# Sudaraka88/LDWeaver

Measured on AMD Instinct MI355X. Metric: MI SNP-pairs/sec, higher is better.
Workload: dtype i8

## Files before the change

ldweaver_amd/csrc/ldw_api.hip:

```cpp
#include <algorithm>
#include <atomic>
#include <chrono>
#include <cmath>
#include <cstdio>
#include <cstdlib>
#include <cstring>

#include <thread>
#include "ldw_internal.h"
#include "ldw_dev.h"
#include "ldw_fasta.h"
#include "ldw_links_read.h"
#include "ldw_slots.h"

namespace ldw {
int check_gpu(ldw_ctx *ctx) {
    LDW_REQUIRE(ctx != nullptr, LDW_ERR_ARG, "null context");
    LDW_HIP(hipSetDevice(ctx->device));
    return LDW_OK;
}
}

using namespace ldw;

// ... 811 lines not shown
            for (int y = 0; y < kb; ++y) {
                const double q = (phi[x] == y ? p[x] : 0.0) + 0.5;
                const double D = p[x] * pY[y] + rxy + p[x] * rX + pY[y] * rY;
                if (!(D > 0.0)) return 1e300;
                F += q * log(q * den / D);
            }
        F /= den;
        if (!(F == F)) return 1e300;
        best = F > best ? F : best;
    }
    return best;
}

__global__ __launch_bounds__(256) void k_snp_sup(int64_t L, const uint32_t *__restrict__ slot_meta, const int64_t *__restrict__ slot_pfix,
                                                 const double *__restrict__ r, double scale, double neff, double r_min, double *__restrict__ sup) {
    const int64_t a = (int64_t)blockIdx.x * 256 + threadIdx.x;
    if (a >= L) return;
    const uint32_t m = slot_meta[a];
    const int n = (int)(m & 7), ka = n + 1;
    double out[4] = {1e300, 1e300, 1e300, 1e300};
    const uint32_t full = (2u << n) - 1u;
    if ((ka == 2 || ka == 3) && ((m >> 3) & full) == full && r[a] == (double)ka) {
        double p[3] = {0.0, 0.0, 0.0};
        double minor = 0.0;
        for (int x = 0; x < ka; ++x) {
            p[x] = (double)slot_pfix[a * 5 + x] * scale;
            if (x < n) minor += p[x];
        }
        if (minor < 0.05 * neff + 4.0)
            for (int kb = 2; kb <= 3; ++kb) {
                out[kb - 2] = mi_vertex_sup(p, ka, kb, neff, 0.25 * ka * kb) * (1.0 + 1e-12) + 1e-12;
                const double rfloor = 0.25 * r_min * r_min;
                out[2 + kb - 2] = mi_vertex_sup(p, ka, kb, neff, rfloor < 0.25 * ka * kb ? rfloor : 0.25 * ka * kb) * (1.0 + 1e-12) + 1e-12;
            }
    }
    for (int k = 0; k < 4; ++k) sup[a * 4 + k] = out[k];
}

static int slot_marginals(ldw_ctx *c, const std::vector<int64_t> &w, int shift, ldw::DevBuf &dst, const char *what) {
    const int64_t L = c->L, Npad = c->Npad;
    ldw::DevBuf d_w, d_p, d_cnt;
    if (int rc = d_w.reserve((size_t)Npad * 8)) return rc;
    if (int rc = d_p.reserve((size_t)L * 40)) return rc;
    if (int rc = d_cnt.reserve((size_t)L * 20)) return rc;
    if (int rc = dst.reserve((size_t)L * 40)) return rc;
    hipError_t he = hipMemcpyAsync(d_w.p, w.data(), (size_t)Npad * 8, hipMemcpyHostToDevice, c->stream);
    hipLaunchKernelGGL(k_counts_marginals, dim3((unsigned)((L + 3) / 4)), dim3(256), 0, c->stream, c->states.as<uint8_t>(), L, Npad, d_w.as<int64_t>(),
                       d_cnt.as<int32_t>(), d_p.as<int64_t>());
    std::vector<int64_t> by_state((size_t)L * 5), by_slot((size_t)L * 5, 0);
    if (he == hipSuccess) he = hipMemcpyAsync(by_state.data(), d_p.p, (size_t)L * 40, hipMemcpyDeviceToHost, c->stream);
    if (he == hipSuccess) he = hipStreamSynchronize(c->stream);
    if (he != hipSuccess) return ldw::hip_fail(he, what, __FILE__, __LINE__);
    for (int64_t a = 0; a < L; ++a) {
        const uint32_t m = c->rows.h_slot_meta[a];
        const int n = (int)(m & 7);
        for (int i = 0; i <= n; ++i) by_slot[a * 5 + i] = by_state[a * 5 + ((m >> (8 + 3 * i)) & 7)] >> shift;
    }
// ... 81 lines not shown
    const int64_t R = c->rows.R;
    lap("slot maps built on the host");
    if (int rc = c->rows.row0.reserve((size_t)(L + 1) * 4)) return rc;
    if (int rc = c->rows.slot_meta.reserve((size_t)L * 4)) return rc;
    if (int rc = c->rows.Mbits.reserve((size_t)(R + TILE) * c->KW * 8)) return rc;
    if (int rc = c->small.reserve((size_t)(R + 1) * 4)) return rc;
    LDW_HIP(hipMemcpyAsync(c->rows.row0.p, c->rows.h_row0.data(), (size_t)(L + 1) * 4, hipMemcpyHostToDevice, c->stream));
    LDW_HIP(hipMemcpyAsync(c->rows.slot_meta.p, meta.data(), (size_t)L * 4, hipMemcpyHostToDevice, c->stream));
    LDW_HIP(hipMemcpyAsync(c->rows.slot_pfix.p, spf.data(), (size_t)L * 40, hipMemcpyHostToDevice, c->stream));
    if (c->apx.apx_ok) {
        if (int rc = slot_marginals(c, c->apx.h_vapx, c->apx.apx_e_last, c->rows.slot_papx, "approximate-weight marginals")) return rc;
    }
    LDW_HIP(hipMemsetAsync(c->rows.Mbits.as<uint64_t>() + (size_t)R * c->KW, 0, (size_t)TILE * c->KW * 8, c->stream));
    lap("approximate marginals");
    if (R > 0) {
        LDW_HIP(hipMemcpyAsync(c->small.p, rowinfo.data(), (size_t)R * 4, hipMemcpyHostToDevice, c->stream));
        LDW_REQUIRE(R < 2147483647LL, LDW_ERR_ARG, "too many indicator rows");
        if (int rc = fill_rows_bits(c, c->small.as<int32_t>(), R)) return rc;
    }
    if (int rc = c->rows.snp_sup.reserve((size_t)L * 32)) return rc;
    hipLaunchKernelGGL(k_snp_sup, dim3((unsigned)((L + 255) / 256)), dim3(256), 0, c->stream, L, c->rows.slot_meta.as<uint32_t>(), c->rows.slot_pfix.as<int64_t>(),
                       c->meta.r.as<double>(), std::ldexp(1.0, -c->wts.frac_bits), c->wts.neff, c->meta.r_min, c->rows.snp_sup.as<double>());
    LDW_HIP(hipGetLastError());
    LDW_HIP(hipStreamSynchronize(c->stream));
    lap("bit rows + per-SNP bounds");
    c->rows_rebuilt();
    return LDW_OK;
}

}
```

ldweaver_amd/csrc/ldw_apx.h:

```cpp
#pragma once
#include "ldw_internal.h"
#include "ldw_epi.h"

namespace ldw {

struct PopSeg {
    uint32_t mask;
    uint32_t flush;
    int64_t V;
};

constexpr int APX_TW = 128;
struct ApxGemmArgs {
    const uint64_t *panel_t, *panel_f;
    int RTpad, RFpad, M2;
    const uint8_t *dig_a, *dig_b;
    const int32_t *shift;
    int32_t *G;
    int lower_only;
    int fine;
    int fuse;
    const uint8_t *bin_t, *bin_f;
    const int2 *tab;
    int tab_nb;
    uint8_t *clean;
    const uint8_t *sr_mask;
    unsigned long long *skip_ctr;
    uint32_t *tile_list;
    unsigned int *n_live;
    int grid_wgs;
    const uint8_t *rflag_t, *rflag_f;
    struct ApxMaybe *maybe;
    unsigned int *maybe_n;
    unsigned int maybe_cap;
};
int launch_pack_panel(ldw_ctx *c, const int32_t *rowlist, int Rpad, uint64_t *panel, hipStream_t st, const int32_t *rowlist2 = nullptr, int Rpad2 = 0,
                      uint64_t *panel2 = nullptr);
int launch_apx_live_tiles(ldw_ctx *c, const ApxGemmArgs &P, hipStream_t st);
int launch_gemm_apx(ldw_ctx *c, const ApxGemmArgs &P, hipStream_t st);
int apx_run_grid(const ldw_ctx *c, int RTpad, int RFpad);
enum PairForm : int { PAIR_FORM_AUTO = 0, PAIR_FORM_QUARTER = 1, PAIR_FORM_WAVE_LDS = 2, PAIR_FORM_WAVE_GLOBAL = 3, PAIR_FORM_BITS = 4 };
struct PairSumsRan {
    int form = 0;
    bool lds160 = false;
};
int launch_pair_sums(ldw_ctx *c, const EpiArgs &A, int64_t *sums, hipStream_t st, int form, int grid_wgs, PairSumsRan *ran);
int launch_pairs_exact(ldw_ctx *c, const EpiArgs &A, unsigned long long *ghist, int64_t *sums, hipStream_t st);

}
```

ldweaver_amd/csrc/ldw_apx.hip:

```cpp
#include <algorithm>
#include <cmath>
#include <cstdlib>
#include <cstring>

#include "ldw_apx.h"
#include "ldw_dev.h"

using namespace ldw;

namespace ldw {

namespace {
constexpr int64_t APX_PROD_CAP = 12000;
struct ProdTable {
    std::vector<int32_t> val;
    std::vector<uint8_t> a, b;
    ProdTable() {
        std::vector<std::pair<int32_t, std::pair<uint8_t, uint8_t>>> all;
        for (int x = 0; x <= 127; ++x)
            for (int y = x; y <= 127; ++y) all.push_back({x * y, {(uint8_t)x, (uint8_t)y}});
        std::sort(all.begin(), all.end());
        for (auto &e : all)
            if (val.empty() || val.back() != e.first) {
                val.push_back(e.first);
// ... 303 lines not shown
            S.fand &= a & 0xFFu;
            S.forr |= o & 0xFFu;
        }
    }
    return S;
}

__global__ __launch_bounds__(256) void k_apx_live_tiles(ApxGemmArgs P) {
    constexpr int MT = APX_MT, NT = 2, TH = 32 * MT, TWd = 32 * NT;
    __shared__ unsigned int s_wave[4], s_base;
    const int ty = (int)blockIdx.x, ntx = P.RFpad / TWd;
    const int lane = threadIdx.x & 63, wave = threadIdx.x >> 6;
    const TileSummary T = apx_fold_rows(P.bin_t + (int64_t)ty * TH, P.rflag_t ? P.rflag_t + (int64_t)ty * TH : nullptr, TH);
    unsigned int n_pruned = 0;
    for (int tx0 = 0; tx0 < ntx; tx0 += 256) {
        const int tx = tx0 + (int)threadIdx.x;
        const bool valid = tx < ntx && !(P.lower_only && tx * TWd + TWd - 1 < ty * TH);
        bool pruned = false, all_binned = false;
        if (valid && !(P.sr_mask && P.sr_mask[(int64_t)((ty * TH) / 128) * (P.RFpad / 64) + tx] != 0)) {
            const TileSummary F = apx_fold_rows(P.bin_f + (int64_t)tx * TWd, P.rflag_f ? P.rflag_f + (int64_t)tx * TWd : nullptr, TWd);
            all_binned = T.bmax < P.tab_nb && F.bmax < P.tab_nb;
            if (P.rflag_t) {
                const unsigned kt = T.fand & PF_KIND, kf = F.fand & PF_KIND;
                pruned = kt >= 2u && kt == (T.forr & PF_KIND) && kf >= 2u && kf == (F.forr & PF_KIND) &&
                         ((T.fand & (kf == 2u ? PF_DEAD2 : PF_DEAD3)) != 0u || (F.fand & (kt == 2u ? PF_DEAD2 : PF_DEAD3)) != 0u);
            }
            if (!pruned && all_binned && (T.bmax - T.bmin + 1) * (F.bmax - F.bmin + 1) <= 64) {
                bool ok = true;
                for (int bt = T.bmin; bt <= T.bmax; ++bt)
                    for (int bf = F.bmin; bf <= F.bmax; ++bf) {
                        const int2 th = P.tab[bt * P.tab_nb + bf];
                        ok = ok && th.x < 0 && th.y == 2147483647;
                    }
                pruned = ok;
            }
        }
        if (pruned && all_binned) {
#pragma unroll
            for (int i = 0; i < MT; ++i)
#pragma unroll
                for (int h = 0; h < (NT * 32) / 64; ++h) P.clean[(int64_t)((ty * TH + 32 * i) / 32) * (P.RFpad / 64) + (tx * TWd) / 64 + h] = 1;
        }
        const bool live = valid && !pruned;
        const unsigned long long lm = __ballot(live);
        n_pruned += (unsigned int)__popcll(__ballot(valid && pruned));
        if (lane == 0) s_wave[wave] = (unsigned int)__popcll(lm);
        __syncthreads();
        if (threadIdx.x == 0) {
// ... 872 lines not shown
```

ldweaver_amd/csrc/ldw_internal.h:

```cpp
#pragma once
#include <hip/hip_runtime.h>
#include <stdint.h>
#include <stdlib.h>
#include <algorithm>
#include <string>
#include <atomic>
#include <chrono>
#include <memory>
#include <mutex>
#include <thread>
#include <vector>

#include "../../include/ldweaver_amd.h"
#include "../../include/ldweaver_amd_debug.h"
#include "ldw_own.h"

#define LDW_NSLOT 3


namespace ldw {

void set_error(const char *fmt, ...);
int hip_fail(hipError_t e, const char *what, const char *file, int line);

// ... 111 lines not shown
        int64_t n_slots = 0;
    } pos_ord;
    void drop() { have_meta = pos_only = false; }
    void mark_set(bool positions_only) { have_meta = true, pos_only = positions_only; }
    void set_positions(const int32_t *POS_, int64_t L) {
        h_POS.assign(POS_, POS_ + L);
        pos_sorted = true;
        for (int64_t i = 1; i < L && pos_sorted; ++i) pos_sorted = POS_[i] >= POS_[i - 1];
        pos_strict = pos_sorted;
        for (int64_t i = 1; i < L && pos_strict; ++i) pos_strict = POS_[i] > POS_[i - 1];
        pos_ord.n_slots = 0;
    }
};

struct SrSizing {
    double sr_total_dist = -1;
    int64_t sr_total = -1;
    uint64_t sr_share_key = 0;
    int64_t sr_share_rows = -1;
    void learn_share(uint64_t key, int64_t n_rows) { sr_share_key = key, sr_share_rows = n_rows; }
    void forget() { sr_total = sr_share_rows = -1, sr_total_dist = -1; }
};

struct OrderCache { std::vector<int32_t> idx, order; };
struct RowMap {
    bool rows_ready = false;
    int64_t R = 0;
    DevBuf Mbits;
    DevBuf row0;
    DevBuf slot_meta;
    DevBuf slot_pfix;
    DevBuf slot_pfix_hi;
    bool hi_ready = false;
    DevBuf slot_papx;
    DevBuf counts;
    DevBuf pfix_state;
    DevBuf snp_sup;
    std::vector<int32_t> h_row0;
    std::vector<uint32_t> h_slot_meta;
    std::vector<int32_t> h_counts;
    std::vector<int64_t> h_minor_w;
    std::vector<int32_t> h_span_bad;
    std::mutex order_mtx;
    std::vector<std::unique_ptr<OrderCache>> order_cache;
    void invalidate() { rows_ready = false; }
    void rebuilt() { rows_ready = true, hi_ready = false, order_cache.clear(); }
};

struct Speculation {
    bool spec_seen[2] = {false, false};
    bool spec_probed[2] = {false, false};
    int spec_hist[2][6] = {{0, 0, 0, 0, 0, 0}, {0, 0, 0, 0, 0, 0}};
    int spec_hist_n[2] = {0, 0};
    bool spec_small[2] = {false, false};
    int spec_B_next[2] = {-1, -1};
    bool maybe_off = false;
    DevBuf tab11[2];
    double tab11_lo[2] = {0, 0};
    int tab11_cur[2] = {0, 0};
    float tab11_c = 0;
// ... 20 lines not shown
};

struct PassCounters {
    int64_t apx_blocks = 0, apx_units_listed = 0, apx_pairs_listed = 0, probe_blocks = 0, generic_blocks = 0;
    int64_t form_launches[5] = {0, 0, 0, 0, 0};
    int64_t pair_kernel_launches[2] = {0, 0};
    int64_t apx_waves_skipped = 0, apx_waves_total = 0;
    int64_t tab11_builds = 0;
    int64_t slot_grown = 0;
    int64_t maybe_entries = 0;
    int64_t pair_list_overflows = 0, maybe_overflows = 0;
    int64_t span_items = 0, span_blocks = 0, span_fallbacks = 0;
    std::atomic<int64_t> sorted_blocks{0};
    int64_t spec_misses = 0, blocks_run = 0, screen_violations = 0, mixed_blocks = 0;
    double gemm_stat[6] = {0, 0, 0, 0, 0, 0};
};

struct Knobs {
    int engine = LDW_ENGINE_MFMA;
    int path_mode = 0;
    int select_mode = 0;
    int mixed = 1;
    bool prune = true;
    bool span_on = true;
    int span_max = 8;
    bool overlap = true;
    int screen = 1;
};

inline bool host_timing() {
    static const bool on = getenv("LDW_HOST_TIMING") != nullptr;
    return on;
}
struct HostClock {
    using Point = std::chrono::steady_clock::time_point;
    static Point now() { return std::chrono::steady_clock::now(); }
    static double ms(Point a, Point b) { return std::chrono::duration<double, std::milli>(b - a).count(); }
    static double us(Point a, Point b) { return std::chrono::duration<double, std::micro>(b - a).count(); }
};
}

struct ldw_ctx {
    int device = 0;
    int n_cu = 0;
    ldw::Stream stream;
    ldw::Stream copy_stream, gemm_stream;
// ... 139 lines not shown
```

ldweaver_amd/csrc/ldw_mi.hip:

```cpp
#include <algorithm>
#include <chrono>
#include <cmath>
#include <cstring>
#include "ldw_prim.h"

#include "ldw_internal.h"
#include "ldw_dev.h"
#ifndef LDW_SCREEN_V
#define LDW_SCREEN_V 2
#endif
#ifndef LDW_SCREEN_WAVES
#define LDW_SCREEN_WAVES 6
#endif
#include "ldw_epi.h"
#include "ldw_pass_plan.h"
#include <future>

#include "ldw_apx.h"

using namespace ldw;

namespace ldw {
#include "ldw_mi_screen.inc"
#include "ldw_mi_eval.inc"
#include "ldw_mi_select.inc"
}

namespace {
#include "ldw_mi_block.inc"
#include "ldw_mi_items.inc"
#include "ldw_mi_pass.inc"
}

namespace ldw {
int ensure_streams(ldw_ctx *c) {
    if (c->streams_ready) return LDW_OK;
    const unsigned quiet = hipEventDisableTiming;
    LDW_HIP(c->copy_stream.ensure(hipStreamNonBlocking));
// ... 124 lines not shown
        if ((rc = c->G.reserve((size_t)RFpad * RTpad * 8))) break;
        for (int pass = 0; pass < 2 && rc == LDW_OK; ++pass) {
            int64_t *host_out = pass == 0 ? counts_out : fixed_out;
            if (!host_out) continue;
            rc = launch_gemm_bits(c, c->rows.Mbits.as<uint64_t>(), c->KW, c->rowlist_t.as<int32_t>(), RTpad, c->rowlist_f.as<int32_t>(), RFpad, c->G.as<int64_t>(),
                                  pass == 0 ? 1 : c->wts.nlimbs, pass == 0 ? d_ones.as<int8_t>() : c->wts.digits.as<int8_t>(), 0);
            if (rc) break;
            hipLaunchKernelGGL(k_tables, dim3((unsigned)((n + 63) / 64)), dim3(64), 0, c->stream, c->G.as<int64_t>(), RFpad,
                               c->idx_f.as<int32_t>(), c->lrow_f.as<int32_t>(), c->idx_t.as<int32_t>(),
                               c->lrow_t.as<int32_t>(), (int)n, c->rows.slot_meta.as<uint32_t>(),
                               pass == 0 ? d_cmarg.as<int64_t>() : c->rows.slot_pfix.as<int64_t>(), d_out.as<int64_t>());
            he = hipMemcpyAsync(host_out + p0 * 25, d_out.p, (size_t)n * 25 * 8, hipMemcpyDeviceToHost, c->stream);
            if (he == hipSuccess) he = hipStreamSynchronize(c->stream);
            if (he != hipSuccess) rc = ldw::hip_fail(he, "joint tables copy", __FILE__, __LINE__);
        }
    }
    return rc;
}

int ldw_links_begin(ldw_ctx *c, int64_t nblocks_capacity) {
    if (int rc = check_gpu(c)) return rc;
    if (int rc = join_prepare(c)) return rc;
    LDW_REQUIRE(nblocks_capacity > 0, LDW_ERR_ARG, "ldw_links_begin: capacity must be positive");
    if (c->links.blk_capacity != 0) {
        if (c->gemm_stream) LDW_HIP(hipStreamSynchronize(c->gemm_stream));
        if (c->copy_stream) LDW_HIP(hipStreamSynchronize(c->copy_stream));
        LDW_HIP(hipStreamSynchronize(c->stream));
        c->links.blk_capacity = 0;
    }
    if (int rc = ensure_rows(c)) return rc;
    const size_t need = 64 + (size_t)LDW_NSLOT * LDW_SPAN_MAX * PICK_STRIDE + (size_t)nblocks_capacity * 32 + 64;
    if (int rc = c->small.reserve(need)) return rc;
    LDW_HIP(hipMemsetAsync(c->small.p, 0, need, c->stream));
    if (int rc = ensure_streams(c)) return rc;
    LDW_HIP(hipEventRecord(c->ev_up[0], c->stream));
    LDW_HIP(hipStreamWaitEvent(c->gemm_stream, c->ev_up[0], 0));
    while ((int64_t)c->ev_pool.size() < nblocks_capacity * EVB) {
        ldw::Event e;
        LDW_HIP(e.ensure());
        c->ev_pool.push_back(std::move(e));
    }
    for (int k = 0; k < LDW_NSLOT; ++k) c->done_recorded[k] = false;
    c->early_sr = false;
    c->ev_valid.assign((size_t)nblocks_capacity, 1);
    c->lrc_recorded = false;
    c->links.new_pass();
// ... 376 lines not shown
```

ldweaver_amd/csrc/ldw_mi_block.inc:

```

int upload_i32(ldw_ctx *c, ldw::DevBuf &buf, const std::vector<int32_t> &v) {
    if (int rc = buf.reserve(v.size() * 4 + 4)) return rc;
    if (!v.empty()) LDW_HIP(hipMemcpyAsync(buf.p, v.data(), v.size() * 4, hipMemcpyHostToDevice, c->stream));
    return LDW_OK;
}

struct SideLists {
    std::vector<int32_t> rowlist, lrow, pos;
    std::vector<uint8_t> cls;
    int Rpad = 0;
};

int build_side(ldw_ctx *c, const int32_t *idx, int64_t n, SideLists &S, const std::vector<int32_t> *order1 = nullptr) {
    S.lrow.assign((size_t)n, 0);
    S.rowlist.clear();
    S.pos.clear();
    S.cls.clear();
    const int32_t zero_row = (int32_t)c->rows.R;
    for (int64_t k = 0; k < n; ++k)
        LDW_REQUIRE(idx[k] >= 0 && idx[k] < c->L, LDW_ERR_ARG, "SNP index %d out of range 0..%lld", idx[k], (long long)c->L - 1);
    for (int cl : {1, 2, 4}) {
        const bool ordered = cl == 1 && order1 != nullptr;
        const int64_t cnt = ordered ? (int64_t)order1->size() : n;
        for (int64_t kk = 0; kk < cnt; ++kk) {
            const int64_t k = ordered ? (int64_t)(*order1)[(size_t)kk] : kk;
            const int32_t a = idx[k];
            const int nr = c->rows.h_row0[a + 1] - c->rows.h_row0[a];
            const int mine = nr <= 1 ? 1 : (nr == 2 ? 2 : 4);
            if (mine != cl) continue;
            S.lrow[k] = (int32_t)S.rowlist.size();
            for (int q = 0; q < cl; ++q) {
                S.rowlist.push_back(q < nr ? c->rows.h_row0[a] + q : zero_row);
                S.pos.push_back(q == 0 ? (int32_t)k : -1);
            }
        }
        while (S.rowlist.size() % 32) {
            S.rowlist.push_back(zero_row);
            S.pos.push_back(-1);
        }
        S.cls.resize(S.rowlist.size() / 32, (uint8_t)cl);
    }
    int64_t rp = ((int64_t)S.rowlist.size() + TILE - 1) / TILE * TILE;
    if (rp == 0) rp = TILE;
    LDW_REQUIRE(rp < 2000000000LL, LDW_ERR_ARG, "block too large");
    S.rowlist.resize((size_t)rp, zero_row);
    S.pos.resize((size_t)rp, -1);
    S.cls.resize((size_t)rp / 32, (uint8_t)1);
    S.Rpad = (int)rp;
// ... 113 lines not shown

struct DevPtrs {
    const int32_t *idx_f, *idx_t, *rl_f, *rl_t, *lrow_f, *lrow_t, *perm, *perm_t, *pos_f, *pos_t;
    const ColInfo *cols;
    const uint8_t *cls_f, *cls_t;
    const int32_t *cmax_f;
    const int64_t *tile_base;
    const int32_t *tf_list;
    const uint8_t *band_mask;
    const uint32_t *band_list;
    int n_band;
    int nf_tiles;
    int gen_t0, gen_q0;
};

struct LoHost {
    int32_t n_lc[3] = {0, 0, 0}, uoff[3] = {0, 0, 0}, rowbase[3] = {0, 0, 0};
    int32_t RTlo = 0, ntiles = 0, n_tf = 0;
    int64_t glo_total = 0;
    int32_t n_tiles_cf[3] = {0, 0, 0};
    int band_full = 0;
    int apx = 0, slot = 0, diag = 0;
    int ordered = 0;
    int fuse_ok = 0;
    int span = 0;
    const SpanSeg *sseg = nullptr;
    mutable const int2 *tab_p = nullptr;
    mutable bool tab_set = false;
};

void fill_epi_args(ldw_ctx *c, const DevPtrs &D, int64_t nf, int64_t nt, int RFpad, int quirk, const EmitArgs &E, const int64_t *G,
                   EpiArgs &A) {
    A.G = G;
    A.mini_c = nullptr;
    A.mini_r = nullptr;
    A.RFpad = RFpad;
    A.RTpad = 0;
    A.idx_f = D.idx_f;
    A.lrow_f = D.lrow_f;
    A.idx_t = D.idx_t;
    A.lrow_t = D.lrow_t;
    A.nf = (int)nf;
    A.nt = (int)nt;
    A.slot_meta = c->rows.slot_meta.as<uint32_t>();
    A.slot_pfix = c->rows.slot_pfix.as<int64_t>();
    A.r = c->meta.r.as<double>();
// ... 366 lines not shown
        ApxGemmArgs P;
        if (E.do_lr) {
            memset(&P, 0, sizeof(P));
            P.panel_f = c->panel[s][0].as<uint64_t>();
            P.panel_t = lo_h->diag ? P.panel_f : c->panel[s][1].as<uint64_t>();
            P.RTpad = RTpad;
            P.RFpad = RFpad;
            P.M2 = (int)(c->KW / 2);
            P.dig_a = c->apx.dig_a.as<uint8_t>();
            P.dig_b = c->apx.dig_b.as<uint8_t>();
            P.shift = c->apx.apx_shift.as<int32_t>();
            P.fine = c->apx.apx_fine ? 1 : 0;
            P.G = c->Gapx[s].as<int32_t>();
            P.lower_only = E.lower_only;
            if (fuse) {
                P.fuse = 1;
                P.skip_ctr = (c->knobs.prune && lo_h->ordered) ? c->apx_skip.as<unsigned long long>() : nullptr;
                if (P.skip_ctr) {
                    P.tile_list = B.tile_list;
                    P.n_live = B.n_live;
                    P.grid_wgs = apx_run_grid(c, RTpad, RFpad);
                    P.rflag_t = rflag_t;
                    P.rflag_f = rflag_f;
                }
                P.bin_t = B.bin_t;
                P.bin_f = B.bin_f;
                P.tab = A.tab11;
                P.tab_nb = A.tab_nb;
                P.clean = c->apx_clean[s].as<uint8_t>();
                P.sr_mask = E.any_sr ? D.band_mask : nullptr;
                if (use_maybe) {
                    P.maybe = maybe_list;
                    P.maybe_n = maybe_n;
                    P.maybe_cap = maybe_cap;
                }
            }
            if (P.skip_ctr)
                if (int rc = launch_apx_live_tiles(c, P, gs)) return rc;
        }
        LDW_HIP(hipEventRecord(ev[0], gs));
        if (E.do_lr)
            if (int rc = launch_gemm_apx(c, P, gs)) return rc;
        LDW_HIP(hipEventRecord(ev[1], gs));
    }
    bind_packs(A, K, true);
    const bool screen_main = c->KW >= swap_kw;
// ... 30 lines not shown
    launch_screen_generic<true>(A, D, (int)egrid.x, U, s2);
    LDW_HIP(hipGetLastError());
    if (need_exact && !band_early)
        if (int rc = launch_gemm_bits(c, c->rows.Mbits.as<uint64_t>(), c->KW, D.rl_t, RTpad, D.rl_f, RFpad, Gx.as<int64_t>(), c->wts.nlimbs, c->wts.digits.as<int8_t>(),
                                      E.lower_only, s2, 0, -1, band, band ? D.band_list : nullptr, D.n_band))
            return rc;
    if (use_pairs) {
        if (int rc = c->pair_sums.reserve((size_t)PAIR_PATHS * PAIR_SHARDS * A.pl_cap * 16 * 8)) return rc;
        if (int rc = launch_pairs_exact(c, A, ghist, c->pair_sums.as<int64_t>(), s2)) return rc;
    }
    if (need_exact) {
        EpiArgs Ax = A;
        Ax.G = Gx.as<int64_t>();
        Ax.E.apx = 0;
        Ax.pl_pairs = nullptr;
        launch_units(Ax, D, U, ghist, s2);
    }
    hipLaunchKernelGGL(k_apx_stats, dim3(1), dim3(64), 0, s2, U.counters, A.pl_n, A.pl_cap, A.E.scr_viol + 1);
    LDW_HIP(hipGetLastError());
    LDW_HIP(hipEventRecord(ev[2], s2));
    return LDW_OK;
}

void build_perm_tiles(ldw_ctx *c, const int32_t *from_idx, int64_t nf, std::vector<int32_t> &perm, const std::vector<int32_t> *order1 = nullptr) {
    perm.clear();
    for (int want : {1, 2, 3, 4, 0}) {
        if (want == 1 && order1) perm.insert(perm.end(), order1->begin(), order1->end());
        else
            for (int64_t k = 0; k < nf; ++k)
                if (c->rows.h_row0[from_idx[k] + 1] - c->rows.h_row0[from_idx[k]] == want) perm.push_back((int32_t)k);
        if (want != 3)
            while (perm.size() % 64) perm.push_back(-1);
    }
    if (perm.empty()) perm.assign(64, -1);
}

void build_perm(ldw_ctx *c, const int32_t *from_idx, int64_t nf, int32_t *perm, const std::vector<int32_t> *order1 = nullptr) {
    int64_t w = 0;
    for (int want : {1, 2, 3, 4, 0}) {
        if (want == 1 && order1) {
            for (int32_t k : *order1) perm[w++] = k;
            continue;
        }
        for (int64_t k = 0; k < nf; ++k)
            if (c->rows.h_row0[from_idx[k] + 1] - c->rows.h_row0[from_idx[k]] == want) perm[w++] = (int32_t)k;
    }
}

const std::vector<int32_t> *minor_weight_order(ldw_ctx *c, const int32_t *idx, int64_t n, std::vector<int32_t> &own) {
    {
        std::lock_guard<std::mutex> lk(c->rows.order_mtx);
        for (auto &pe : c->rows.order_cache)
            if ((int64_t)pe->idx.size() == n && pe->idx[0] == idx[0] && memcmp(pe->idx.data(), idx, (size_t)n * 4) == 0) return &pe->order;
    }
    std::vector<std::pair<int64_t, int32_t>> key;
    key.reserve((size_t)n);
    for (int64_t k = 0; k < n; ++k)
        if (c->rows.h_row0[idx[k] + 1] - c->rows.h_row0[idx[k]] == 1) key.emplace_back(c->rows.h_minor_w[(size_t)idx[k]], (int32_t)k);
    std::sort(key.begin(), key.end());
    own.resize(key.size());
    for (size_t i = 0; i < key.size(); ++i) own[i] = key[i].second;
    std::lock_guard<std::mutex> lk(c->rows.order_mtx);
    if (c->rows.order_cache.size() >= 256) return &own;
    c->rows.order_cache.emplace_back(new ldw::OrderCache());
    auto &e = *c->rows.order_cache.back();
    e.idx.assign(idx, idx + n);
    e.order = own;
    return &e.order;
}

int run_block_mi(ldw_ctx *c, const int32_t *from_idx, int64_t nf, const int32_t *to_idx, int64_t nt, int quirk,
                 EmitArgs E) {
    if (int rc = join_prepare(c)) return rc;
    if (int rc = ensure_rows(c)) return rc;
    LDW_REQUIRE(nf > 0 && nt > 0, LDW_ERR_ARG, "empty block (nf=%lld nt=%lld)", (long long)nf, (long long)nt);
    LDW_REQUIRE(nf <= 1000000 && nt <= 1000000, LDW_ERR_ARG, "block side too long");
    std::vector<int32_t> vf(from_idx, from_idx + nf), vt(to_idx, to_idx + nt), perm, perm_t((size_t)nt);
    SideLists SF, ST;
    if (int rc = build_side(c, from_idx, nf, SF)) return rc;
    if (int rc = build_side(c, to_idx, nt, ST)) return rc;
    build_perm_tiles(c, from_idx, nf, perm);
    build_perm(c, to_idx, nt, perm_t.data());
    if (int rc = upload_i32(c, c->perm_t, perm_t)) return rc;
    if (int rc = upload_i32(c, c->idx_f, vf)) return rc;
    if (int rc = upload_i32(c, c->idx_t, vt)) return rc;
    if (int rc = upload_i32(c, c->rowlist_f, SF.rowlist)) return rc;
    if (int rc = upload_i32(c, c->rowlist_t, ST.rowlist)) return rc;
    if (int rc = upload_i32(c, c->lrow_f, SF.lrow)) return rc;
    if (int rc = upload_i32(c, c->lrow_t, ST.lrow)) return rc;
    if (int rc = upload_i32(c, c->perm_f, perm)) return rc;
    if (int rc = c->hist[0].reserve((size_t)NBINS * 8)) return rc;
// ... 50 lines not shown
```

ldweaver_amd/csrc/ldw_mi_items.inc:

```

struct StageImage {
    struct Part {
        size_t off, bytes;
        const void *src;
        void (*point)(DevPtrs &, const char *);
    };
    Part part[18] = {};
    int n = 0;
    size_t bytes = 0;
    template <class T> static T elem_of(const T *DevPtrs::*);
    template <auto F> using Elem = decltype(elem_of(F));
    template <auto F> size_t array(const Elem<F> *src, size_t count) {
        part[n] = Part{bytes, count * sizeof(Elem<F>), src, [](DevPtrs &D, const char *p) { D.*F = reinterpret_cast<const Elem<F> *>(p); }};
        bytes = (bytes + part[n].bytes + 63) / 64 * 64;
        return part[n++].off;
    }
    void copy_to(char *image) const {
        for (int k = 0; k < n; ++k)
            if (part[k].src && part[k].bytes) memcpy(image + part[k].off, part[k].src, part[k].bytes);
    }
    void bind(DevPtrs &D, const char *image) const {
        for (int k = 0; k < n; ++k) part[k].point(D, image + part[k].off);
    }
};
// ... 25 lines not shown
    int64_t sr_base = 0;
    std::vector<int32_t> span_from, span_to;
};

struct SpanPlan {
    int nseg = 0;
    int32_t start[LDW_SPAN_MAX] = {}, nt[LDW_SPAN_MAX] = {};
};

static inline bool speculation_pays(const ldw_ctx *c, const ldw_mi_params *p) {
    if (c->knobs.path_mode != 0) return true;
    return !(p->lr_links_approx > 0.0) || p->lr_retain_links < 0.007 * p->lr_links_approx;
}

struct PrepWork {
    ldw_ctx *c;
    const int32_t *from_idx, *to_idx;
    int64_t nf, nt;
    HostBlock &hb;
    std::vector<ColInfo> cols;
    std::string cols_err;
    std::future<int> cols_job;
    const std::vector<int32_t> *ord_f = nullptr, *ord_t = nullptr;
    std::vector<int32_t> ord_f_own, ord_t_own, ord_f_full, ord_t_full;
    SideLists SF, ST;
    std::vector<int32_t> pf, cmax, tf;
    std::vector<int64_t> tbase;
    std::vector<uint8_t> band;
    std::vector<uint32_t> bandl;
    int intervals(const ldw_mi_params *p, const SpanPlan *sp);
    int row_order(const SpanPlan *sp);
    void tiles(int slot);
    void band_mask();
    bool band_list();
    int join_cols() {
        const int rc = cols_job.valid() ? cols_job.get() : LDW_OK;
        if (rc != LDW_OK) set_error("%s", cols_err.c_str());
        return rc;
    }
    ~PrepWork() { if (cols_job.valid()) cols_job.wait(); }
};

int PrepWork::intervals(const ldw_mi_params *p, const SpanPlan *sp) {
    const int64_t blk_no = hb.blk_no;
    auto ascending = [&](const int32_t *idx, int64_t n) {
        for (int64_t k = 1; k < n; ++k)
            if (c->meta.h_POS[idx[k]] < c->meta.h_POS[idx[k - 1]]) return false;
        return true;
    };
    hb.generic = !ascending(from_idx, nf) || !ascending(to_idx, nt);
    if (hb.generic) {
        ColInfo z;
        memset(&z, 0, sizeof(z));
        cols.assign((size_t)nt, z);
// ... 13 lines not shown
        cols_job = std::async(std::launch::async, [this, sr_dist]() -> int {
            const int rc = build_cols(c, from_idx, nf, to_idx, nt, true, sr_dist, cols, hb.n_sr_blk);
            if (rc != LDW_OK) cols_err = ldw_last_error();
            return rc;
        });
    } else if (int rc = build_cols(c, from_idx, nf, to_idx, nt, hb.diag, p->sr_dist, cols, hb.n_sr_blk)) return rc;
    if (sp) {
        LDW_REQUIRE(!hb.generic && !hb.diag && sp->nseg >= 1 && sp->nseg <= LDW_SPAN_MAX, LDW_ERR_STATE,
                    "span of %d blocks at block %lld cannot be formed", sp->nseg, (long long)blk_no);
        hb.span = sp->nseg;
        for (int k = 0; k < sp->nseg; ++k) {
            hb.seg_start[k] = sp->start[k];
            hb.seg_nt[k] = sp->nt[k];
            hb.seg_lr_total[k] = nf * (int64_t)sp->nt[k] - std::min<int64_t>(nf, sp->nt[k]);
            for (int32_t b = sp->start[k]; b < sp->start[k] + sp->nt[k]; ++b) {
                cols[(size_t)b].pad[0] = k;
                cols[(size_t)b].pad[1] = sp->start[k];
            }
        }
    }
    return LDW_OK;
}

int PrepWork::row_order(const SpanPlan *sp) {
    if (c->knobs.prune && !hb.generic && !hb.diag && c->knobs.engine == LDW_ENGINE_MFMA && c->apx.apx_ok) {
        bool rowless = false;
        for (int64_t k = 0; k < nf && !rowless; ++k) rowless = c->rows.h_row0[from_idx[k] + 1] == c->rows.h_row0[from_idx[k]];
        for (int64_t k = 0; k < nt && !rowless; ++k) rowless = c->rows.h_row0[to_idx[k] + 1] == c->rows.h_row0[to_idx[k]];
        if (!rowless) {
            ord_f = minor_weight_order(c, from_idx, nf, ord_f_full);
            ord_t = minor_weight_order(c, to_idx, nt, ord_t_full);
            if (hb.n_sr_blk > 0) {
                std::vector<int32_t> df((size_t)nf + 1, 0);
                std::vector<uint8_t> in_f((size_t)nf, 0), in_t((size_t)nt, 0);
                for (int64_t b = 0; b < nt; ++b)
                    for (int iv = 0; iv < 3; ++iv) {
                        const ColInfo &ci = cols[(size_t)b];
                        if (ci.e[iv] <= ci.s[iv]) continue;
                        in_t[(size_t)b] = 1;
                        ++df[(size_t)ci.s[iv]];
                        --df[(size_t)ci.e[iv]];
                    }
                int32_t run = 0;
                for (int64_t a = 0; a < nf; ++a) {
                    run += df[(size_t)a];
                    in_f[(size_t)a] = run > 0 ? 1 : 0;
                }
                auto rest_then_corner = [&](const std::vector<int32_t> &sorted, const std::vector<uint8_t> &corner, const int32_t *idx, int64_t n,
                                            std::vector<int32_t> &out) {
                    out.clear();
                    out.reserve(sorted.size());
                    for (int32_t k : sorted)
                        if (!corner[(size_t)k]) out.push_back(k);
                    for (int64_t k = 0; k < n; ++k)
                        if (corner[(size_t)k] && c->rows.h_row0[idx[k] + 1] - c->rows.h_row0[idx[k]] == 1) out.push_back((int32_t)k);
                };
                rest_then_corner(*ord_f, in_f, from_idx, nf, ord_f_own);
                rest_then_corner(*ord_t, in_t, to_idx, nt, ord_t_own);
                ord_f = &ord_f_own;
                ord_t = &ord_t_own;
            }
            c->cnt.sorted_blocks += sp ? sp->nseg : 1;
        }
    }
    LDW_REQUIRE(!sp || (ord_f && ord_t), LDW_ERR_STATE, "span at block %lld cannot be ordered", (long long)hb.blk_no);
    return LDW_OK;
}

void PrepWork::tiles(int slot) {
    build_perm_tiles(c, from_idx, nf, pf, ord_f);
    hb.D.nf_tiles = (int)(pf.size() / 64);
    {
        int64_t n12f = 0, n1 = 0, n2 = 0;
        for (int64_t k = 0; k < nf; ++k) {
            const int nr = c->rows.h_row0[from_idx[k] + 1] - c->rows.h_row0[from_idx[k]];
            n1 += nr == 1;
            n2 += nr == 2;
        }
        n12f = (n1 + 63) / 64 + (n2 + 63) / 64;
        hb.D.gen_t0 = (int)n12f;
        int64_t q12 = 0;
        for (int64_t k = 0; k < nt; ++k) {
            const int nr = c->rows.h_row0[to_idx[k] + 1] - c->rows.h_row0[to_idx[k]];
            q12 += nr == 1 || nr == 2;
        }
        hb.D.gen_q0 = (int)q12;
    }
    cmax.assign((size_t)hb.D.nf_tiles, 1);
    tbase.assign(cmax.size(), 0);
    {
        LoHost &lo = hb.lo;
        lo = LoHost();
        for (int64_t k = 0; k < nt; ++k) ++lo.n_lc[lo_class(c->rows.h_row0[to_idx[k] + 1] - c->rows.h_row0[to_idx[k]])];
// ... 81 lines not shown
                    if (ci.e[iv] <= ci.s[iv]) continue;
                    for (int k = 0; k < 3; ++k) {
                        const int32_t n0 = pre[k][(size_t)ci.s[iv]], n1 = pre[k][(size_t)ci.e[iv]];
                        if (n1 <= n0) continue;
                        int64_t f0 = base[k] + (int64_t)(n0 / 64 * 64) * (1 << k), f1 = base[k] + (int64_t)((n1 + 63) / 64 * 64) * (1 << k);
                        if (k == 0 && ord_f) {
                            const int64_t first = nxt1[(size_t)ci.s[iv]], last = prv1[(size_t)ci.e[iv]];
                            f0 = (int64_t)SF.lrow[(size_t)first] / 64 * 64;
                            f1 = ((int64_t)SF.lrow[(size_t)last] + 1 + 63) / 64 * 64;
                        }
                        if (k == 2) {
                            f0 = base[2];
                            f1 = base[2] + (int64_t)pre[2][(size_t)nf] * 4;
                        }
                        if (f1 > hb.RFpad) f1 = hb.RFpad;
                        mark(rb0, rb1, f0, f1);
                        if (hb.diag) mark(f0, f1, rb0, rb1);
                    }
                }
            }
    }
    hb.lo.fuse_ok = no_rowless ? 1 : 0;
    hb.lo.ordered = ord_f != nullptr ? 1 : 0;
}

bool PrepWork::band_list() {
    bool listed = false;
    const int64_t ntx = hb.RFpad / 64;
    if (hb.n_sr_blk > 0 && !hb.lo.band_full && hb.RTpad / TILE < 65536 && ntx < 65536) {
        const int64_t nty = hb.RTpad / TILE;
        for (int64_t ty = 0; ty < nty; ++ty)
            for (int64_t tx = 0; tx < ntx; ++tx)
                if (band[(size_t)ty * ntx + tx] && !(hb.diag && tx * 64 + 63 < ty * TILE)) bandl.push_back((uint32_t)(ty << 16 | tx));
        listed = bandl.size() * 2 <= band.size();
        if (!listed) bandl.clear();
    }
    hb.D.n_band = (int)bandl.size();
    return listed;
}

int prep_block(ldw_ctx *c, const int32_t *from_idx, int64_t nf, const int32_t *to_idx, int64_t nt, const ldw_mi_params *p,
               int slot, int64_t blk_no, HostBlock &hb, const SpanPlan *sp = nullptr, int pin_slot = -1, size_t stage_base = 0) {
    LDW_REQUIRE(nf > 0 && nt > 0, LDW_ERR_ARG, "empty block (nf=%lld nt=%lld)", (long long)nf, (long long)nt);
    LDW_REQUIRE(nf <= 1000000 && nt <= 1000000 && nf * nt < 2147483647LL, LDW_ERR_ARG, "block too large (%lld x %lld)",
                (long long)nf, (long long)nt);
    for (int64_t k = 0; k < nf; ++k)
        LDW_REQUIRE(from_idx[k] >= 0 && from_idx[k] < c->L, LDW_ERR_ARG, "SNP index %d out of range", from_idx[k]);
    for (int64_t k = 0; k < nt; ++k)
        LDW_REQUIRE(to_idx[k] >= 0 && to_idx[k] < c->L, LDW_ERR_ARG, "SNP index %d out of range", to_idx[k]);
    const bool prep_timing = ldw::host_timing();
    auto pnow = [] { return std::chrono::duration<double, std::micro>(std::chrono::steady_clock::now().time_since_epoch()).count(); };
    double tp[8] = {pnow(), 0, 0, 0, 0, 0, 0, 0};
    hb = HostBlock();
    hb.nf = nf;
    hb.nt = nt;
    hb.slot = slot;
    hb.blk_no = blk_no;
    hb.pin_slot = pin_slot;
    hb.stage_base = stage_base;
    hb.diag = same_list(from_idx, nf, to_idx, nt);
    PrepWork W{c, from_idx, to_idx, nf, nt, hb};
    if (int rc = W.intervals(p, sp)) return rc;
    tp[1] = pnow();
    if (int rc = W.row_order(sp)) return rc;
    tp[2] = pnow();
    if (int rc = build_side(c, from_idx, nf, W.SF, W.ord_f)) return rc;
    if (int rc = build_side(c, to_idx, nt, W.ST, W.ord_t)) return rc;
    tp[3] = pnow();
    hb.RFpad = W.SF.Rpad;
    hb.RTpad = W.ST.Rpad;
    W.tiles(slot);
    if (int rc = W.join_cols()) return rc;
    hb.n_lr_total = (hb.diag ? nf * (nf - 1) / 2 : nf * nt - std::min(nf, nt)) - hb.n_sr_blk;
    tp[4] = pnow();
    W.band_mask();
    tp[5] = pnow();
    const bool band_listed = W.band_list();
    StageImage &im = hb.img;
    im.array<&DevPtrs::idx_f>(from_idx, (size_t)nf);
    im.array<&DevPtrs::idx_t>(to_idx, (size_t)nt);
    im.array<&DevPtrs::rl_f>(W.SF.rowlist.data(), W.SF.rowlist.size());
    im.array<&DevPtrs::rl_t>(W.ST.rowlist.data(), W.ST.rowlist.size());
    im.array<&DevPtrs::lrow_f>(W.SF.lrow.data(), (size_t)nf);
    im.array<&DevPtrs::lrow_t>(W.ST.lrow.data(), (size_t)nt);
    im.array<&DevPtrs::perm>(W.pf.data(), W.pf.size());
    const size_t at_perm_t = im.array<&DevPtrs::perm_t>(nullptr, (size_t)nt);
    im.array<&DevPtrs::cols>(W.cols.data(), W.cols.size());
    im.array<&DevPtrs::pos_f>(W.SF.pos.data(), W.SF.pos.size());
    im.array<&DevPtrs::pos_t>(W.ST.pos.data(), W.ST.pos.size());
    im.array<&DevPtrs::cls_f>(W.SF.cls.data(), W.SF.cls.size());
    im.array<&DevPtrs::cls_t>(W.ST.cls.data(), W.ST.cls.size());
    im.array<&DevPtrs::cmax_f>(W.cmax.data(), W.cmax.size());
    im.array<&DevPtrs::tile_base>(W.tbase.data(), W.tbase.size());
    im.array<&DevPtrs::tf_list>(W.tf.data(), W.tf.size());
    im.array<&DevPtrs::band_mask>(W.band.data(), W.band.size());
    if (band_listed) im.array<&DevPtrs::band_list>(W.bandl.data(), W.bandl.size());
    hb.total = im.bytes;
    const int ps = pin_slot >= 0 ? pin_slot : slot;
    if (c->pin[ps].cap < stage_base + hb.total)
        if (int rc = c->pin[ps].reserve_keep((stage_base + hb.total) * 2, stage_base)) return rc;
    tp[6] = pnow();
    char *b = c->pin[ps].as<char>() + stage_base;
    im.copy_to(b);
    build_perm(c, to_idx, nt, reinterpret_cast<int32_t *>(b + at_perm_t), W.ord_t);
    if (prep_timing && blk_no < 12)
        fprintf(stderr, "[ldw prep us] block %lld%s %lld x %lld span %d: checks + intervals %.0f  row order %.0f  sides %.0f  tiles + classes %.0f  band %.0f  band list %.0f  copy to staging %.0f  (%zu bytes)\n",
                (long long)blk_no, hb.diag ? " diag" : "", (long long)nf, (long long)nt, hb.span, tp[1] - tp[0], tp[2] - tp[1], tp[3] - tp[2], tp[4] - tp[3], tp[5] - tp[4], tp[6] - tp[5], pnow() - tp[6], hb.total);
    return LDW_OK;
}

int launch_gather(ldw_ctx *c, const HostBlock &hb, const EmitArgs &E, const SmallLayout &sl) {
    GatherArgs S;
    S.MI = c->MIblk.as<double>();
    S.cols = E.cols;
    S.nf = (int)hb.nf;
    S.nt = (int)hb.nt;
    S.lower_only = E.lower_only;
    hipLaunchKernelGGL(k_lr_gather, dim3((unsigned)((hb.nt + 15) / 16)), dim3(256), 0, c->stream, S, sl.pick[hb.slot], E.ckey, E.cval);
    LDW_HIP(hipGetLastError());
    return LDW_OK;
}

double lo_bound(const ldw_ctx *c) {
    const double den = c->wts.neff > 1.0 ? c->wts.neff : 1.0;
    return c->wts.lo_abs_sum * (2.0 * std::log(den + 12.5) + 3.0) / den;
}

// ... 646 lines not shown
```

Measured before the change: 178.1 billion.

## Order two-row SNPs by MI bound and refine tile pruning on folded rows

Copies per-SNP MI upper bounds to the host and uses them to sort two-row SNPs within each block side, so SNPs with similar bounds land in the same tiles. This reordering is only enabled by an environment variable. The approximate GEMM live-tile check also re-folds flags over the aligned 128-row span of the from side to detect dead kind-3 tiles, and the per-SNP bound kernel drops its minor-weight gate so more SNPs get finite bounds. It adds a device-to-host copy, a host sort, and extra folding work in the tile filter in exchange for more tiles that can be skipped.

```diff
diff --git a/ldweaver_amd/csrc/ldw_api.hip b/ldweaver_amd/csrc/ldw_api.hip
--- a/ldweaver_amd/csrc/ldw_api.hip
+++ b/ldweaver_amd/csrc/ldw_api.hip
@@ -857,17 +857,12 @@
     const uint32_t full = (2u << n) - 1u;
     if ((ka == 2 || ka == 3) && ((m >> 3) & full) == full && r[a] == (double)ka) {
         double p[3] = {0.0, 0.0, 0.0};
-        double minor = 0.0;
-        for (int x = 0; x < ka; ++x) {
-            p[x] = (double)slot_pfix[a * 5 + x] * scale;
-            if (x < n) minor += p[x];
-        }
-        if (minor < 0.05 * neff + 4.0)
-            for (int kb = 2; kb <= 3; ++kb) {
-                out[kb - 2] = mi_vertex_sup(p, ka, kb, neff, 0.25 * ka * kb) * (1.0 + 1e-12) + 1e-12;
-                const double rfloor = 0.25 * r_min * r_min;
-                out[2 + kb - 2] = mi_vertex_sup(p, ka, kb, neff, rfloor < 0.25 * ka * kb ? rfloor : 0.25 * ka * kb) * (1.0 + 1e-12) + 1e-12;
-            }
+        for (int x = 0; x < ka; ++x) p[x] = (double)slot_pfix[a * 5 + x] * scale;
+        for (int kb = 2; kb <= 3; ++kb) {
+            out[kb - 2] = mi_vertex_sup(p, ka, kb, neff, 0.25 * ka * kb) * (1.0 + 1e-12) + 1e-12;
+            const double rfloor = 0.25 * r_min * r_min;
+            out[2 + kb - 2] = mi_vertex_sup(p, ka, kb, neff, rfloor < 0.25 * ka * kb ? rfloor : 0.25 * ka * kb) * (1.0 + 1e-12) + 1e-12;
+        }
     }
     for (int k = 0; k < 4; ++k) sup[a * 4 + k] = out[k];
 }
@@ -995,6 +990,8 @@
     hipLaunchKernelGGL(k_snp_sup, dim3((unsigned)((L + 255) / 256)), dim3(256), 0, c->stream, L, c->rows.slot_meta.as<uint32_t>(), c->rows.slot_pfix.as<int64_t>(),
                        c->meta.r.as<double>(), std::ldexp(1.0, -c->wts.frac_bits), c->wts.neff, c->meta.r_min, c->rows.snp_sup.as<double>());
     LDW_HIP(hipGetLastError());
+    c->rows.h_snp_sup.resize((size_t)L * 4);
+    LDW_HIP(hipMemcpyAsync(c->rows.h_snp_sup.data(), c->rows.snp_sup.p, (size_t)L * 32, hipMemcpyDeviceToHost, c->stream));
     LDW_HIP(hipStreamSynchronize(c->stream));
     lap("bit rows + per-SNP bounds");
     c->rows_rebuilt();
diff --git a/ldweaver_amd/csrc/ldw_apx.h b/ldweaver_amd/csrc/ldw_apx.h
--- a/ldweaver_amd/csrc/ldw_apx.h
+++ b/ldweaver_amd/csrc/ldw_apx.h
@@ -30,6 +30,7 @@
     unsigned int *n_live;
     int grid_wgs;
     const uint8_t *rflag_t, *rflag_f;
+    int f2_row0;
     struct ApxMaybe *maybe;
     unsigned int *maybe_n;
     unsigned int maybe_cap;
diff --git a/ldweaver_amd/csrc/ldw_apx.hip b/ldweaver_amd/csrc/ldw_apx.hip
--- a/ldweaver_amd/csrc/ldw_apx.hip
+++ b/ldweaver_amd/csrc/ldw_apx.hip
@@ -349,8 +349,16 @@
             all_binned = T.bmax < P.tab_nb && F.bmax < P.tab_nb;
             if (P.rflag_t) {
                 const unsigned kt = T.fand & PF_KIND, kf = F.fand & PF_KIND;
-                pruned = kt >= 2u && kt == (T.forr & PF_KIND) && kf >= 2u && kf == (F.forr & PF_KIND) &&
-                         ((T.fand & (kf == 2u ? PF_DEAD2 : PF_DEAD3)) != 0u || (F.fand & (kt == 2u ? PF_DEAD2 : PF_DEAD3)) != 0u);
+                const bool kinds = kt >= 2u && kt == (T.forr & PF_KIND) && kf >= 2u && kf == (F.forr & PF_KIND);
+                unsigned f_dead = F.fand;
+                if (kinds && kf == 3u && (T.fand & PF_DEAD3) == 0u && (F.fand & (kt == 2u ? PF_DEAD2 : PF_DEAD3)) != 0u) {
+                    const int r0 = tx * TWd - P.f2_row0;
+                    const int lo = P.f2_row0 + r0 / 128 * 128;
+                    int hi = P.f2_row0 + (r0 + TWd + 127) / 128 * 128;
+                    hi = hi < P.RFpad ? hi : P.RFpad;
+                    f_dead = r0 >= 0 ? apx_fold_rows(P.bin_f + lo, P.rflag_f + lo, hi - lo).fand : 0u;
+                }
+                pruned = kinds && ((T.fand & (kf == 2u ? PF_DEAD2 : PF_DEAD3)) != 0u || (f_dead & (kt == 2u ? PF_DEAD2 : PF_DEAD3)) != 0u);
             }
             if (!pruned && all_binned && (T.bmax - T.bmin + 1) * (F.bmax - F.bmin + 1) <= 64) {
                 bool ok = true;
diff --git a/ldweaver_amd/csrc/ldw_internal.h b/ldweaver_amd/csrc/ldw_internal.h
--- a/ldweaver_amd/csrc/ldw_internal.h
+++ b/ldweaver_amd/csrc/ldw_internal.h
@@ -157,7 +157,8 @@
     void forget() { sr_total = sr_share_rows = -1, sr_total_dist = -1; }
 };
 
-struct OrderCache { std::vector<int32_t> idx, order; };
+struct RowOrders { std::vector<int32_t> one, two[2]; };
+struct OrderCache { std::vector<int32_t> idx; RowOrders ord; };
 struct RowMap {
     bool rows_ready = false;
     int64_t R = 0;
@@ -171,6 +172,7 @@
     DevBuf counts;
     DevBuf pfix_state;
     DevBuf snp_sup;
+    std::vector<double> h_snp_sup;
     std::vector<int32_t> h_row0;
     std::vector<uint32_t> h_slot_meta;
     std::vector<int32_t> h_counts;
@@ -237,6 +239,7 @@
     int select_mode = 0;
     int mixed = 1;
     bool prune = true;
+    bool row2_order = false;
     bool span_on = true;
     int span_max = 8;
     bool overlap = true;
diff --git a/ldweaver_amd/csrc/ldw_mi.hip b/ldweaver_amd/csrc/ldw_mi.hip
--- a/ldweaver_amd/csrc/ldw_mi.hip
+++ b/ldweaver_amd/csrc/ldw_mi.hip
@@ -14,6 +14,7 @@
 #endif
 #include "ldw_epi.h"
 #include "ldw_pass_plan.h"
+#include "ldw_row_order.h"
 #include <future>
 
 #include "ldw_apx.h"
@@ -184,6 +185,7 @@
     if (int rc = check_gpu(c)) return rc;
     if (int rc = join_prepare(c)) return rc;
     LDW_REQUIRE(nblocks_capacity > 0, LDW_ERR_ARG, "ldw_links_begin: capacity must be positive");
+    c->knobs.row2_order = getenv("LDW_ROW2_ORDER") != nullptr;
     if (c->links.blk_capacity != 0) {
         if (c->gemm_stream) LDW_HIP(hipStreamSynchronize(c->gemm_stream));
         if (c->copy_stream) LDW_HIP(hipStreamSynchronize(c->copy_stream));
diff --git a/ldweaver_amd/csrc/ldw_mi_block.inc b/ldweaver_amd/csrc/ldw_mi_block.inc
--- a/ldweaver_amd/csrc/ldw_mi_block.inc
+++ b/ldweaver_amd/csrc/ldw_mi_block.inc
@@ -11,7 +11,8 @@
     int Rpad = 0;
 };
 
-int build_side(ldw_ctx *c, const int32_t *idx, int64_t n, SideLists &S, const std::vector<int32_t> *order1 = nullptr) {
+int build_side(ldw_ctx *c, const int32_t *idx, int64_t n, SideLists &S, const std::vector<int32_t> *order1 = nullptr,
+               const std::vector<int32_t> *order2 = nullptr) {
     S.lrow.assign((size_t)n, 0);
     S.rowlist.clear();
     S.pos.clear();
@@ -20,10 +21,10 @@
     for (int64_t k = 0; k < n; ++k)
         LDW_REQUIRE(idx[k] >= 0 && idx[k] < c->L, LDW_ERR_ARG, "SNP index %d out of range 0..%lld", idx[k], (long long)c->L - 1);
     for (int cl : {1, 2, 4}) {
-        const bool ordered = cl == 1 && order1 != nullptr;
-        const int64_t cnt = ordered ? (int64_t)order1->size() : n;
+        const std::vector<int32_t> *order = cl == 1 ? order1 : (cl == 2 ? order2 : nullptr);
+        const int64_t cnt = order ? (int64_t)order->size() : n;
         for (int64_t kk = 0; kk < cnt; ++kk) {
-            const int64_t k = ordered ? (int64_t)(*order1)[(size_t)kk] : kk;
+            const int64_t k = order ? (int64_t)(*order)[(size_t)kk] : kk;
             const int32_t a = idx[k];
             const int nr = c->rows.h_row0[a + 1] - c->rows.h_row0[a];
             const int mine = nr <= 1 ? 1 : (nr == 2 ? 2 : 4);
@@ -183,6 +184,7 @@
     int band_full = 0;
     int apx = 0, slot = 0, diag = 0;
     int ordered = 0;
+    int f2_row0 = 0;
     int fuse_ok = 0;
     int span = 0;
     const SpanSeg *sseg = nullptr;
@@ -595,6 +597,7 @@
                     P.grid_wgs = apx_run_grid(c, RTpad, RFpad);
                     P.rflag_t = rflag_t;
                     P.rflag_f = rflag_f;
+                    P.f2_row0 = lo_h->f2_row0;
                 }
                 P.bin_t = B.bin_t;
                 P.bin_f = B.bin_f;
@@ -671,10 +674,12 @@
     return LDW_OK;
 }
 
-void build_perm_tiles(ldw_ctx *c, const int32_t *from_idx, int64_t nf, std::vector<int32_t> &perm, const std::vector<int32_t> *order1 = nullptr) {
+void build_perm_tiles(ldw_ctx *c, const int32_t *from_idx, int64_t nf, std::vector<int32_t> &perm, const std::vector<int32_t> *order1 = nullptr,
+                      const std::vector<int32_t> *order2 = nullptr) {
     perm.clear();
     for (int want : {1, 2, 3, 4, 0}) {
-        if (want == 1 && order1) perm.insert(perm.end(), order1->begin(), order1->end());
+        const std::vector<int32_t> *order = want == 1 ? order1 : (want == 2 ? order2 : nullptr);
+        if (order) perm.insert(perm.end(), order->begin(), order->end());
         else
             for (int64_t k = 0; k < nf; ++k)
                 if (c->rows.h_row0[from_idx[k] + 1] - c->rows.h_row0[from_idx[k]] == want) perm.push_back((int32_t)k);
@@ -684,11 +689,12 @@
     if (perm.empty()) perm.assign(64, -1);
 }
 
-void build_perm(ldw_ctx *c, const int32_t *from_idx, int64_t nf, int32_t *perm, const std::vector<int32_t> *order1 = nullptr) {
+void build_perm(ldw_ctx *c, const int32_t *from_idx, int64_t nf, int32_t *perm, const std::vector<int32_t> *order1 = nullptr,
+                const std::vector<int32_t> *order2 = nullptr) {
     int64_t w = 0;
     for (int want : {1, 2, 3, 4, 0}) {
-        if (want == 1 && order1) {
-            for (int32_t k : *order1) perm[w++] = k;
+        if (const std::vector<int32_t> *order = want == 1 ? order1 : (want == 2 ? order2 : nullptr)) {
+            for (int32_t k : *order) perm[w++] = k;
             continue;
         }
         for (int64_t k = 0; k < nf; ++k)
@@ -696,26 +702,35 @@
     }
 }
 
-const std::vector<int32_t> *minor_weight_order(ldw_ctx *c, const int32_t *idx, int64_t n, std::vector<int32_t> &own) {
+const ldw::RowOrders *list_row_orders(ldw_ctx *c, const int32_t *idx, int64_t n, ldw::RowOrders &own) {
     {
         std::lock_guard<std::mutex> lk(c->rows.order_mtx);
         for (auto &pe : c->rows.order_cache)
-            if ((int64_t)pe->idx.size() == n && pe->idx[0] == idx[0] && memcmp(pe->idx.data(), idx, (size_t)n * 4) == 0) return &pe->order;
+            if ((int64_t)pe->idx.size() == n && pe->idx[0] == idx[0] && memcmp(pe->idx.data(), idx, (size_t)n * 4) == 0) return &pe->ord;
     }
     std::vector<std::pair<int64_t, int32_t>> key;
+    std::vector<int32_t> two;
     key.reserve((size_t)n);
-    for (int64_t k = 0; k < n; ++k)
-        if (c->rows.h_row0[idx[k] + 1] - c->rows.h_row0[idx[k]] == 1) key.emplace_back(c->rows.h_minor_w[(size_t)idx[k]], (int32_t)k);
+    for (int64_t k = 0; k < n; ++k) {
+        const int nr = c->rows.h_row0[idx[k] + 1] - c->rows.h_row0[idx[k]];
+        if (nr == 1) key.emplace_back(c->rows.h_minor_w[(size_t)idx[k]], (int32_t)k);
+        else if (nr == 2) two.push_back((int32_t)k);
+    }
     std::sort(key.begin(), key.end());
-    own.resize(key.size());
-    for (size_t i = 0; i < key.size(); ++i) own[i] = key[i].second;
+    own.one.resize(key.size());
+    for (size_t i = 0; i < key.size(); ++i) own.one[i] = key[i].second;
+    std::vector<double> bound(two.size());
+    for (int m = 0; m < 2; ++m) {
+        for (size_t i = 0; i < two.size(); ++i) bound[i] = c->rows.h_snp_sup[(size_t)idx[two[i]] * 4 + 2 * m];
+        ldw::order_by_bound(two, bound, own.two[m]);
+    }
     std::lock_guard<std::mutex> lk(c->rows.order_mtx);
     if (c->rows.order_cache.size() >= 256) return &own;
     c->rows.order_cache.emplace_back(new ldw::OrderCache());
     auto &e = *c->rows.order_cache.back();
     e.idx.assign(idx, idx + n);
-    e.order = own;
-    return &e.order;
+    e.ord = own;
+    return &e.ord;
 }
 
 int run_block_mi(ldw_ctx *c, const int32_t *from_idx, int64_t nf, const int32_t *to_idx, int64_t nt, int quirk,
diff --git a/ldweaver_amd/csrc/ldw_mi_items.inc b/ldweaver_amd/csrc/ldw_mi_items.inc
--- a/ldweaver_amd/csrc/ldw_mi_items.inc
+++ b/ldweaver_amd/csrc/ldw_mi_items.inc
@@ -71,14 +71,16 @@
     std::string cols_err;
     std::future<int> cols_job;
     const std::vector<int32_t> *ord_f = nullptr, *ord_t = nullptr;
-    std::vector<int32_t> ord_f_own, ord_t_own, ord_f_full, ord_t_full;
+    const std::vector<int32_t> *ord2_f = nullptr, *ord2_t = nullptr;
+    std::vector<int32_t> ord_f_own, ord_t_own;
+    ldw::RowOrders ord_f_full, ord_t_full;
     SideLists SF, ST;
     std::vector<int32_t> pf, cmax, tf;
     std::vector<int64_t> tbase;
     std::vector<uint8_t> band;
     std::vector<uint32_t> bandl;
     int intervals(const ldw_mi_params *p, const SpanPlan *sp);
-    int row_order(const SpanPlan *sp);
+    int row_order(const ldw_mi_params *p, const SpanPlan *sp);
     void tiles(int slot);
     void band_mask();
     bool band_list();
@@ -138,14 +140,20 @@
     return LDW_OK;
 }
 
-int PrepWork::row_order(const SpanPlan *sp) {
+int PrepWork::row_order(const ldw_mi_params *p, const SpanPlan *sp) {
     if (c->knobs.prune && !hb.generic && !hb.diag && c->knobs.engine == LDW_ENGINE_MFMA && c->apx.apx_ok) {
         bool rowless = false;
         for (int64_t k = 0; k < nf && !rowless; ++k) rowless = c->rows.h_row0[from_idx[k] + 1] == c->rows.h_row0[from_idx[k]];
         for (int64_t k = 0; k < nt && !rowless; ++k) rowless = c->rows.h_row0[to_idx[k] + 1] == c->rows.h_row0[to_idx[k]];
         if (!rowless) {
-            ord_f = minor_weight_order(c, from_idx, nf, ord_f_full);
-            ord_t = minor_weight_order(c, to_idx, nt, ord_t_full);
+            const ldw::RowOrders *of = list_row_orders(c, from_idx, nf, ord_f_full), *ot = list_row_orders(c, to_idx, nt, ord_t_full);
+            ord_f = &of->one;
+            ord_t = &ot->one;
+            if (hb.n_sr_blk == 0 && c->knobs.row2_order) {
+                const int m = p->quirk_mode == LDW_QUIRK_REFERENCE ? 1 : 0;
+                ord2_f = &of->two[m];
+                ord2_t = &ot->two[m];
+            }
             if (hb.n_sr_blk > 0) {
                 std::vector<int32_t> df((size_t)nf + 1, 0);
                 std::vector<uint8_t> in_f((size_t)nf, 0), in_t((size_t)nt, 0);
@@ -184,7 +192,7 @@
 }
 
 void PrepWork::tiles(int slot) {
-    build_perm_tiles(c, from_idx, nf, pf, ord_f);
+    build_perm_tiles(c, from_idx, nf, pf, ord_f, ord2_f);
     hb.D.nf_tiles = (int)(pf.size() / 64);
     {
         int64_t n12f = 0, n1 = 0, n2 = 0;
@@ -312,6 +320,12 @@
     }
     hb.lo.fuse_ok = no_rowless ? 1 : 0;
     hb.lo.ordered = ord_f != nullptr ? 1 : 0;
+    hb.lo.f2_row0 = 0;
+    for (size_t g = 0; g < SF.cls.size(); ++g)
+        if (SF.cls[g] == 2) {
+            hb.lo.f2_row0 = (int)(g * 32);
+            break;
+        }
 }
 
 bool PrepWork::band_list() {
@@ -352,10 +366,10 @@
     PrepWork W{c, from_idx, to_idx, nf, nt, hb};
     if (int rc = W.intervals(p, sp)) return rc;
     tp[1] = pnow();
-    if (int rc = W.row_order(sp)) return rc;
+    if (int rc = W.row_order(p, sp)) return rc;
     tp[2] = pnow();
-    if (int rc = build_side(c, from_idx, nf, W.SF, W.ord_f)) return rc;
-    if (int rc = build_side(c, to_idx, nt, W.ST, W.ord_t)) return rc;
+    if (int rc = build_side(c, from_idx, nf, W.SF, W.ord_f, W.ord2_f)) return rc;
+    if (int rc = build_side(c, to_idx, nt, W.ST, W.ord_t, W.ord2_t)) return rc;
     tp[3] = pnow();
     hb.RFpad = W.SF.Rpad;
     hb.RTpad = W.ST.Rpad;
@@ -392,7 +406,7 @@
     tp[6] = pnow();
     char *b = c->pin[ps].as<char>() + stage_base;
     im.copy_to(b);
-    build_perm(c, to_idx, nt, reinterpret_cast<int32_t *>(b + at_perm_t), W.ord_t);
+    build_perm(c, to_idx, nt, reinterpret_cast<int32_t *>(b + at_perm_t), W.ord_t, W.ord2_t);
     if (prep_timing && blk_no < 12)
         fprintf(stderr, "[ldw prep us] block %lld%s %lld x %lld span %d: checks + intervals %.0f  row order %.0f  sides %.0f  tiles + classes %.0f  band %.0f  band list %.0f  copy to staging %.0f  (%zu bytes)\n",
                 (long long)blk_no, hb.diag ? " diag" : "", (long long)nf, (long long)nt, hb.span, tp[1] - tp[0], tp[2] - tp[1], tp[3] - tp[2], tp[4] - tp[3], tp[5] - tp[4], tp[6] - tp[5], pnow() - tp[6], hb.total);
diff --git a/ldweaver_amd/csrc/ldw_row_order.h b/ldweaver_amd/csrc/ldw_row_order.h
--- /dev/null
+++ b/ldweaver_amd/csrc/ldw_row_order.h
@@ -0,0 +1,25 @@
+#pragma once
+#include <algorithm>
+#include <cstdint>
+#include <vector>
+
+namespace ldw {
+
+constexpr double SNP_SUP_NONE = 1e300;
+inline bool bound_is_finite(double key) { return key < SNP_SUP_NONE; }
+
+inline void order_by_bound(const std::vector<int32_t> &members, const std::vector<double> &key, std::vector<int32_t> &out) {
+    const size_t n = members.size() < key.size() ? members.size() : key.size();
+    std::vector<uint32_t> at;
+    at.reserve(n);
+    for (size_t i = 0; i < n; ++i)
+        if (bound_is_finite(key[i])) at.push_back((uint32_t)i);
+    std::stable_sort(at.begin(), at.end(), [&](uint32_t x, uint32_t y) { return key[x] < key[y]; });
+    out.clear();
+    out.reserve(n);
+    for (uint32_t i : at) out.push_back(members[i]);
+    for (size_t i = 0; i < n; ++i)
+        if (!bound_is_finite(key[i])) out.push_back(members[i]);
+}
+
+}
```

After: 172.8 billion. 3.0% lower.
